# ryogrid/anime-illust-image-searcher

Measured on AMD Instinct MI355X. Metric: images/sec tagged (ViT fwd), higher is better.
Workload: dtype f16; 1 GPU; wd-tagger ViT-B/16 448px 16-bit-operand forward + sigmoid + MCut tag selection, batch 64 per GPU, u8 NHWC images resident in HBM (BASELINE.json configs[1]); batch_per_gpu=64, image=448x448x3 u8, classes=10861, parallelism=single GPU

## Files before the change

anime-illust-image-searcher_amd/csrc/vit.hip:

```cpp
#include <algorithm>
#include "../../include/hip_tagsearch_debug.h"
#include <cmath>
#include <cstdlib>
#include <cstdio>
#include <cstring>
#include <string>
#include <vector>

#include "vit_internal.h"
#include "model_host.h"

using namespace hipts;

namespace {

struct Layer {
    DevBuf ln1_g, ln1_b, ln2_g, ln2_b;
    DevBuf qkv_w, qkv_b, proj_w, proj_b, fc1_w, fc1_b, fc2_w, fc2_b;
    DevBuf qkv_u, qkv_c, fc1_u, fc1_c;
};


}

enum ProfCat { PC_PATCHIFY = 0, PC_GEMM_PATCH, PC_LAYERNORM, PC_GEMM_QK, PC_GEMM_VT, PC_ATTENTION, PC_GEMM_RESID,
               PC_GEMM_GELU, PC_POOL, PC_GEMM_HEAD, PC_OTHER, PC_COUNT };
static_assert(PC_COUNT == HIPTS_VIT_PROF_CATEGORIES, "category count");
static const char* const kProfNames[PC_COUNT] = {
    "patchify_kernel", "gemm_kernel<EPI_PATCH>", "layernorm_kernel", "gemm_kernel<EPI_QKV>", "gemm_kernel<EPI_VT>",
    "attn2_kernel", "gemm_kernel<EPI_RESID>", "gemm_kernel<EPI_GELU>", "pool_kernels", "gemm_kernel<EPI_HEAD>", "other"};

struct ProfRec {
    int cat;
    hipEvent_t a, b;
    double flops, bytes;
};

struct hipts_vit {
    bool prof = false;
    int prof_every = 0;
    uint32_t prof_mask = 0xffffffffu;
    long prof_calls = 0;
    std::vector<ProfRec> recs;
    std::vector<hipEvent_t> pool;
    double acc_ms[PC_COUNT] = {0}, acc_flops[PC_COUNT] = {0}, acc_bytes[PC_COUNT] = {0};
    int64_t acc_n[PC_COUNT] = {0};
    int device = 0;
    hipts_vit_config_t cfg{};
    int grid = 0, tokens = 0, tokens_pad = 0, patch_k = 0;
    std::vector<Layer> layers;
    DevBuf patch_w, patch_w2, patch_b, patch_b_u8, pos, norm_g, norm_b, head_w, head_b;
    std::vector<float> h_patch_bias, h_patch_rowsum;
    TensorLedger ledger;
    DevBuf img_in, a0, x, xn, q, k, v, att, hmid, pool_part, pooled2, logits, probs, stat_part;
    DevBuf x_rm;
    DevBuf sk_ws;
    bool fold_ln = false;
    bool fold_dirty = true;
    bool split_att = false;
    int pool_splits = 1;
    static constexpr int kMaxSub = 4;
    int want_sub = 0;
    bool deferred_join = false;
    int last_ns = 0;
    int pend_ns = 0, pend_batch = 0;
    SubStreams<kMaxSub> streams;
    hipEvent_t ev_stagger = nullptr;
};

namespace {

template <bool F16>
__global__ __launch_bounds__(256) void patchify_u8_kernel(const uint8_t* __restrict__ img, bf16_t* __restrict__ a0, int batch,
                                                          int size, int P, int grid) {
    const int64_t idx = (int64_t)blockIdx.x * 256 + threadIdx.x;
    const int64_t total = (int64_t)batch * grid * grid * P;
    if (idx >= total) return;
    const int ky = (int)(idx % P);
    const int64_t tok = idx / P;
    const int px = (int)(tok % grid), py = (int)((tok / grid) % grid), b = (int)(tok / ((int64_t)grid * grid));
    const uint8_t* src = img + (((int64_t)b * size + (py * P + ky)) * size + px * P) * 3;
    bf16_t* dst = a0 + tok * (int64_t)(P * P * 3) + ky * P * 3;
    if (P == 16) {
        const uint4* s4 = reinterpret_cast<const uint4*>(src);
        uint4* d4 = reinterpret_cast<uint4*>(dst);
#pragma unroll
        for (int v = 0; v < 3; ++v) {
            const uint4 in = s4[v];
            const uint32_t w[4] = {in.x, in.y, in.z, in.w};
            bf16x8 lo, hi;
#pragma unroll
            for (int e = 0; e < 8; ++e) {
                lo[e] = to_op<F16>((float)((w[e >> 2] >> (8 * (e & 3))) & 0xffu));
                hi[e] = to_op<F16>((float)((w[2 + (e >> 2)] >> (8 * (e & 3))) & 0xffu));
            }
            d4[2 * v] = *reinterpret_cast<const uint4*>(&lo);
            d4[2 * v + 1] = *reinterpret_cast<const uint4*>(&hi);
        }
        return;
    }
    for (int i = 0; i < P * 3; ++i) dst[i] = to_op<F16>((float)src[i]);
}

template <bool F16>
__global__ __launch_bounds__(256) void patchify_u8_p16_kernel(const uint8_t* __restrict__ img, bf16_t* __restrict__ a0, int size, int grid,
                                                              int xgroups) {
    __shared__ __attribute__((aligned(16))) char image[16 * 1536];
    const int tid = threadIdx.x;
    const int xg = blockIdx.x % xgroups, py = (blockIdx.x / xgroups) % grid, b = blockIdx.x / (xgroups * grid);
    const int px0 = xg * 16, ntok = min(16, grid - px0);
    const int chunks_per_row = ntok * 3;
    const int total = 16 * chunks_per_row;
    const uint8_t* src0 = img + (((int64_t)b * size + (int64_t)py * 16) * size + px0 * 16) * 3;
#pragma unroll
    for (int j = 0; j < 3; ++j) {
        const int L = j * 256 + tid;
        if (L < total) {
            const int ky = L / chunks_per_row, c16 = L - ky * chunks_per_row;
            const uint4 in = *reinterpret_cast<const uint4*>(src0 + (int64_t)ky * size * 3 + c16 * 16);
            const uint32_t w[4] = {in.x, in.y, in.z, in.w};
            bf16x8 lo, hi;
#pragma unroll
            for (int e = 0; e < 8; ++e) {
                lo[e] = to_op<F16>((float)((w[e >> 2] >> (8 * (e & 3))) & 0xffu));
                hi[e] = to_op<F16>((float)((w[2 + (e >> 2)] >> (8 * (e & 3))) & 0xffu));
            }
            const int tok = c16 / 3, part = c16 - tok * 3;
            char* d = image + tok * 1536 + ky * 96 + part * 32;
            *reinterpret_cast<bf16x8*>(d) = lo;
            *reinterpret_cast<bf16x8*>(d + 16) = hi;
        }
    }
    __syncthreads();
    const int out_chunks = ntok * 96;
    uint4* dst = reinterpret_cast<uint4*>(a0 + (((int64_t)b * grid + py) * grid + px0) * 768);
    for (int L = tid; L < out_chunks; L += 256) dst[L] = *reinterpret_cast<const uint4*>(image + L * 16);
}

template <bool F16>
__global__ __launch_bounds__(256) void patchify_f32_kernel(const float* __restrict__ x, bf16_t* __restrict__ a0, int batch,
                                                           int size, int P, int grid) {
    const int64_t idx = (int64_t)blockIdx.x * 256 + threadIdx.x;
    const int64_t total = (int64_t)batch * grid * grid * P;
    if (idx >= total) return;
    const int ky = (int)(idx % P);
    const int64_t tok = idx / P;
    const int px = (int)(tok % grid), py = (int)((tok / grid) % grid), b = (int)(tok / ((int64_t)grid * grid));
    const int K = P * P * 3;
    bf16_t* dst = a0 + tok * (int64_t)(2 * K) + ky * P * 3;
    for (int c = 0; c < 3; ++c) {
        const float* src = x + (((int64_t)b * 3 + (2 - c)) * size + (py * P + ky)) * size + px * P;
        for (int kx = 0; kx < P; ++kx) {
            const float v = src[kx];
            const bf16_t hi = to_op<F16>(v);
            dst[kx * 3 + c] = hi;
            dst[K + kx * 3 + c] = to_op<F16>(v - from_op<F16>(hi));
        }
    }
}

__device__ __forceinline__ float wave_sum(float v) {
#pragma unroll
    for (int o = 32; o >= 1; o >>= 1) v += __shfl_xor(v, o);
    return v;
}

template <bool F16, bool OUT8 = false>
__global__ __launch_bounds__(256) void layernorm_kernel(const float* __restrict__ x, const float* __restrict__ g,
                                                        const float* __restrict__ bta, bf16_t* __restrict__ out, int64_t rows,
                                                        int D, float eps) {
    const int lane = threadIdx.x & 63;
    const int64_t row = (int64_t)blockIdx.x * 4 + (threadIdx.x >> 6);
    if (row >= rows) return;
    const int nvec = D >> 2;
    const float4* xr = reinterpret_cast<const float4*>(x + row * D);
    float4 v[4];
    float s = 0.f;
#pragma unroll
    for (int i = 0; i < 4; ++i) {
        const int c = lane + 64 * i;
        v[i] = c < nvec ? xr[c] : make_float4(0.f, 0.f, 0.f, 0.f);
        s += (v[i].x + v[i].y) + (v[i].z + v[i].w);
    }
    const float mean = wave_sum(s) / (float)D;
    float ss = 0.f;
#pragma unroll
    for (int i = 0; i < 4; ++i) {
        if (lane + 64 * i < nvec) {
            const float a = v[i].x - mean, b = v[i].y - mean, c = v[i].z - mean, d = v[i].w - mean;
            ss += (a * a + b * b) + (c * c + d * d);
        }
    }
    const float rstd = 1.0f / sqrtf(wave_sum(ss) / (float)D + eps);
    const float4* gr = reinterpret_cast<const float4*>(g);
    const float4* br = reinterpret_cast<const float4*>(bta);
#pragma unroll
    for (int i = 0; i < 4; ++i) {
        const int c = lane + 64 * i;
        if (c < nvec) {
            const float4 gg = gr[c], bb = bta ? br[c] : make_float4(0.f, 0.f, 0.f, 0.f);
            if constexpr (OUT8)
                reinterpret_cast<uint32_t*>(reinterpret_cast<uint8_t*>(out) + row * D)[c] =
                    pack4_e4m3((v[i].x - mean) * rstd * gg.x + bb.x, (v[i].y - mean) * rstd * gg.y + bb.y,
                               (v[i].z - mean) * rstd * gg.z + bb.z, (v[i].w - mean) * rstd * gg.w + bb.w);
            else
            *reinterpret_cast<bf16x4*>(out + row * D + 4 * c) =
                pack4<F16>((v[i].x - mean) * rstd * gg.x + bb.x, (v[i].y - mean) * rstd * gg.y + bb.y,
                           (v[i].z - mean) * rstd * gg.z + bb.z, (v[i].w - mean) * rstd * gg.w + bb.w);
        }
    }
}

__global__ __launch_bounds__(256) void pool_partial_kernel(const float* __restrict__ x, float* __restrict__ part, int tokens,
                                                           int D, float eps, int normalize, int splits) {
    __shared__ float red[4][1024];
    const int lane = threadIdx.x & 63, wave = threadIdx.x >> 6;
    const int split = blockIdx.x, b = blockIdx.y;
    const int per = (tokens + splits - 1) / splits;
    const int t0 = split * per, t1 = min(tokens, t0 + per);
    const int nvec = D >> 2;
    float4 acc[4];
#pragma unroll
    for (int i = 0; i < 4; ++i) acc[i] = make_float4(0.f, 0.f, 0.f, 0.f);
    auto load_row = [&](int t, float4 (&v)[4]) {
        const float4* xr = reinterpret_cast<const float4*>(x + ((int64_t)b * tokens + (t < t1 ? t : t1 - 1)) * D);
#pragma unroll
        for (int i = 0; i < 4; ++i) {
            const int c = lane + 64 * i;
            v[i] = c < nvec ? xr[c] : make_float4(0.f, 0.f, 0.f, 0.f);
        }
    };
    float4 vn[4];
    if (t0 + wave < t1) load_row(t0 + wave, vn);
    for (int t = t0 + wave; t < t1; t += 4) {
        float4 v[4];
        float s = 0.f;
#pragma unroll
        for (int i = 0; i < 4; ++i) {
            v[i] = vn[i];
            s += (v[i].x + v[i].y) + (v[i].z + v[i].w);
        }
        if (t + 4 < t1) load_row(t + 4, vn);
        float mean = 0.f, rstd = 1.f;
        if (normalize) {
            mean = wave_sum(s) / (float)D;
            float ss = 0.f;
#pragma unroll
            for (int i = 0; i < 4; ++i)
                if (lane + 64 * i < nvec) {
                    const float a = v[i].x - mean, bq = v[i].y - mean, c = v[i].z - mean, d = v[i].w - mean;
                    ss += (a * a + bq * bq) + (c * c + d * d);
                }
            rstd = 1.0f / sqrtf(wave_sum(ss) / (float)D + eps);
        }
#pragma unroll
        for (int i = 0; i < 4; ++i) {
            acc[i].x += (v[i].x - mean) * rstd;
            acc[i].y += (v[i].y - mean) * rstd;
            acc[i].z += (v[i].z - mean) * rstd;
            acc[i].w += (v[i].w - mean) * rstd;
        }
    }
#pragma unroll
    for (int i = 0; i < 4; ++i) {
        const int c = lane + 64 * i;
        if (c < nvec) {
            red[wave][4 * c + 0] = acc[i].x;
            red[wave][4 * c + 1] = acc[i].y;
            red[wave][4 * c + 2] = acc[i].z;
            red[wave][4 * c + 3] = acc[i].w;
        }
    }
    __syncthreads();
    for (int d = threadIdx.x; d < D; d += 256)
        part[((int64_t)b * splits + split) * D + d] = (red[0][d] + red[1][d]) + (red[2][d] + red[3][d]);
}

template <bool F16>
__global__ __launch_bounds__(256) void pool_finalize_kernel(const float* __restrict__ part, const float* __restrict__ g,
                                                            const float* __restrict__ bta, bf16_t* __restrict__ out, int tokens,
                                                            int D, float eps, int normalize_after, int splits) {
    __shared__ float feat[1024];
    __shared__ float red[8];
    const int b = blockIdx.x;
    float s = 0.f;
    for (int d = threadIdx.x; d < D; d += 256) {
        float a = 0.f;
        for (int sp = 0; sp < splits; ++sp) a += part[((int64_t)b * splits + sp) * D + d];
        a = a / (float)tokens;
        feat[d] = a;
        s += a;
    }
    float mean = 0.f, rstd = 1.f;
    if (normalize_after) {
        s = wave_sum(s);
        if ((threadIdx.x & 63) == 0) red[threadIdx.x >> 6] = s;
        __syncthreads();
        mean = ((red[0] + red[1]) + (red[2] + red[3])) / (float)D;
        float ss = 0.f;
        for (int d = threadIdx.x; d < D; d += 256) {
            const float c = feat[d] - mean;
            ss += c * c;
        }
        ss = wave_sum(ss);
        if ((threadIdx.x & 63) == 0) red[4 + (threadIdx.x >> 6)] = ss;
        __syncthreads();
        rstd = 1.0f / sqrtf(((red[4] + red[5]) + (red[6] + red[7])) / (float)D + eps);
    }
    for (int d = threadIdx.x; d < D; d += 256) {
        const float f = (feat[d] - mean) * rstd * g[d] + bta[d];
        const bf16_t hi = to_op<F16>(f);
        const bf16_t lo = to_op<F16>(f - from_op<F16>(hi));
        out[(int64_t)b * 2 * D + d] = hi;
        out[(int64_t)b * 2 * D + D + d] = lo;
    }
}

}

extern "C" {

int hipts_vit_create(const hipts_vit_config_t* cfg, int device, hipts_vit_t** out) {
    HIPTS_REQUIRE(cfg && out, "hipts_vit_create: null argument");
    HIPTS_REQUIRE(cfg->patch >= 4 && cfg->image_size % cfg->patch == 0, "image_size must be a multiple of patch");
    HIPTS_REQUIRE(cfg->heads >= 1 && cfg->dim == cfg->heads * 64, "head dim must be 64 (dim = heads * 64)");
    HIPTS_REQUIRE(cfg->dim % 64 == 0 && cfg->dim <= 1024, "dim must be a multiple of 64, <= 1024");
    HIPTS_REQUIRE(cfg->mlp_dim % 64 == 0, "mlp_dim must be a multiple of 64");
    HIPTS_REQUIRE((cfg->patch * cfg->patch * 3) % 64 == 0, "patch*patch*3 must be a multiple of 64");
    HIPTS_REQUIRE(cfg->depth >= 1 && cfg->num_classes >= 1 && cfg->max_batch >= 1, "bad depth / classes / max_batch");
    const int grid = cfg->image_size / cfg->patch;
    HIPTS_REQUIRE((grid * grid) % 4 == 0, "token count must be a multiple of 4");
    HIPTS_TRY(use_device(device));
    auto* h = new hipts_vit();
    h->device = device;
    h->cfg = *cfg;
    h->grid = grid;
    h->tokens = grid * grid;
    h->tokens_pad = round_up(h->tokens, 64);
    h->patch_k = cfg->patch * cfg->patch * 3;
    h->split_att = (cfg->operand_f16 & HIPTS_OPERAND_SPLIT_ATT) != 0;
    h->layers.resize(cfg->depth);
    for (const char* s : {"patch_embed.proj.weight", "patch_embed.proj.bias", "pos_embed", "norm.weight", "norm.bias", "head.weight", "head.bias"})
        h->ledger.need(s);
    for (int i = 0; i < cfg->depth; ++i) {
        const std::string p = "blocks." + std::to_string(i) + ".";
        for (const char* s : {"norm1.weight", "norm1.bias", "attn.qkv.weight", "attn.qkv.bias", "attn.proj.weight",
                              "attn.proj.bias", "norm2.weight", "norm2.bias", "mlp.fc1.weight", "mlp.fc1.bias",
                              "mlp.fc2.weight", "mlp.fc2.bias"})
            h->ledger.need(p + s);
    }
    const size_t B = cfg->max_batch, M = B * h->tokens, D = cfg->dim;
    const size_t qkv_elems = B * cfg->heads * (size_t)h->tokens_pad * 64;
    h->pool_splits = h->tokens >= 64 ? std::min(32, std::max(8, h->tokens / 28)) : 1;
    if (getenv("HIPTS_POOL_SPLITS") && h->tokens >= 64) h->pool_splits = std::max(1, std::min(32, atoi(getenv("HIPTS_POOL_SPLITS"))));
    int st = HIPTS_OK;
    if ((st = h->a0.alloc(M * h->patch_k * 2 * 2)) || (st = h->x.alloc(M * D * 4)) || (st = h->x_rm.alloc(M * D * 4)) || (st = h->xn.alloc(M * D * 2)) ||
        (st = h->q.alloc(qkv_elems * 2)) || (st = h->k.alloc(qkv_elems * 2)) || (st = h->v.alloc(qkv_elems * 2)) ||
        (st = h->att.alloc(M * D * 2 * (h->split_att ? 2 : 1))) || (st = h->hmid.alloc(M * (size_t)cfg->mlp_dim * 2)) ||
        (st = h->pool_part.alloc(B * h->pool_splits * D * 4)) || (st = h->pooled2.alloc(B * 2 * D * 2)) ||
        (st = h->logits.alloc(B * (size_t)cfg->num_classes * 4)) || (st = h->probs.alloc(B * (size_t)cfg->num_classes * 4))) {
        delete h;
        return st;
    }
    h->fold_ln = D % 64 == 0 && h->tokens % 8 == 0 && cfg->mlp_dim % 8 == 0 && !getenv("HIPTS_GEMM") &&
                 !(getenv("HIPTS_LN_FOLD") && atoi(getenv("HIPTS_LN_FOLD")) == 0);
    if (h->fold_ln) {
        if ((st = h->stat_part.alloc(((D + 255) / 256) * M * 8))) {
            delete h;
            return st;
        }
        for (auto& L : h->layers)
            if ((st = L.qkv_u.alloc(3 * D * 4)) || (st = L.qkv_c.alloc(3 * D * 4)) || (st = L.fc1_u.alloc((size_t)cfg->mlp_dim * 4)) ||
                (st = L.fc1_c.alloc((size_t)cfg->mlp_dim * 4))) {
                delete h;
                return st;
            }
    }
    {
        hipError_t e2;
        if ((st = h->sk_ws.alloc(hipts_vit::kMaxSub * GEMM_SK_WS_BYTES)) || (e2 = hipMemset(h->sk_ws.p, 0, h->sk_ws.bytes)) != hipSuccess) {
            delete h;
            return st ? st : set_error(HIPTS_ERR_HIP, "hipMemset failed");
        }
    }
    hipError_t e;
    if ((e = hipMemset(h->q.p, 0, h->q.bytes)) != hipSuccess || (e = hipMemset(h->k.p, 0, h->k.bytes)) != hipSuccess ||
        (e = hipMemset(h->v.p, 0, h->v.bytes)) != hipSuccess) {
        delete h;
        return set_error(HIPTS_ERR_HIP, "hipMemset failed: %s", hipGetErrorString(e));
    }
    *out = h;
    return HIPTS_OK;
}

int hipts_vit_destroy(hipts_vit_t* h) {
    if (h) {
        (void)hipSetDevice(h->device);
        (void)hipDeviceSynchronize();
        if (h->ev_stagger) (void)hipEventDestroy(h->ev_stagger);
        delete h;
    }
    return HIPTS_OK;
}

int hipts_vit_set_tensor(hipts_vit_t* h, const char* key_c, const float* data, int64_t numel) {
    HIPTS_REQUIRE(h && key_c && data, "hipts_vit_set_tensor: null argument");
    HIPTS_TRY(use_device(h->device));
    const bool f16 = (h->cfg.operand_f16 & 1) != 0;
    const std::string key(key_c);
    const auto& c = h->cfg;
    const int D = c.dim, P = c.patch, Mlp = c.mlp_dim, C = c.num_classes;
#define EXPECT(n)                                                                                                      \
    HIPTS_REQUIRE(numel == (int64_t)(n), "tensor %s: expected %lld elements, got %lld", key_c, (long long)(n),         \
                  (long long)numel)
    int st = HIPTS_ERR_INVALID, li = 0;
    std::string sub;
    if (key == "patch_embed.proj.weight") {
        EXPECT((int64_t)D * 3 * P * P);
        std::vector<float> perm((size_t)D * h->patch_k);
        for (int n = 0; n < D; ++n)
            for (int ky = 0; ky < P; ++ky)
                for (int kx = 0; kx < P; ++kx)
                    for (int cr = 0; cr < 3; ++cr)
                        perm[(size_t)n * h->patch_k + (ky * P + kx) * 3 + cr] = data[(((size_t)n * 3 + (2 - cr)) * P + ky) * P + kx];
        st = upload_matrix16(h->patch_w, perm.data(), D, h->patch_k, round_up(D, 256), f16);
        if (st == HIPTS_OK) {
            h->h_patch_rowsum.assign(D, 0.f);
            for (int n = 0; n < D; ++n) {
                double rs = 0.0;
                for (int kk = 0; kk < h->patch_k; ++kk) {
                    float wv;
                    if (f16) {
                        wv = f16_bits_to_f32(f32_to_f16_rne(perm[(size_t)n * h->patch_k + kk]));
                    } else {
                        const uint32_t bits = (uint32_t)f32_to_bf16_rne(perm[(size_t)n * h->patch_k + kk]) << 16;
                        memcpy(&wv, &bits, 4);
                    }
                    rs += (double)wv;
                }
                h->h_patch_rowsum[n] = (float)rs;
            }
            st = upload_matrix16_dup(h->patch_w2, perm.data(), D, h->patch_k, round_up(D, 256), f16);
        }
    } else if (key == "patch_embed.proj.bias") {
        EXPECT(D);
        h->h_patch_bias.assign(data, data + D);
        st = upload_f32(h->patch_b, data, D);
    } else if (key == "pos_embed") {
        EXPECT((int64_t)h->tokens * D);
        st = upload_f32(h->pos, data, (size_t)h->tokens * D);
    } else if (key == "norm.weight") {
        EXPECT(D);
        st = upload_f32(h->norm_g, data, D);
    } else if (key == "norm.bias") {
        EXPECT(D);
        st = upload_f32(h->norm_b, data, D);
    } else if (key == "head.weight") {
        EXPECT((int64_t)C * D);
        st = upload_matrix16_dup(h->head_w, data, C, D, round_up(C, 256), f16);
    } else if (key == "head.bias") {
        EXPECT(C);
        st = upload_f32(h->head_b, data, C);
    } else if (parse_indexed(key, "blocks.", &li, &sub)) {
        HIPTS_REQUIRE(li >= 0 && li < c.depth, "tensor %s: block index out of range", key_c);
        Layer& L = h->layers[li];
        if (sub == "norm1.weight") { EXPECT(D); st = upload_f32(L.ln1_g, data, D); }
        else if (sub == "norm1.bias") { EXPECT(D); st = upload_f32(L.ln1_b, data, D); }
        else if (sub == "norm2.weight") { EXPECT(D); st = upload_f32(L.ln2_g, data, D); }
        else if (sub == "norm2.bias") { EXPECT(D); st = upload_f32(L.ln2_b, data, D); }
        else if (sub == "attn.qkv.weight") { EXPECT((int64_t)3 * D * D); st = upload_matrix16(L.qkv_w, data, 3 * D, D, round_up(2 * D, 256) + round_up(D, 256) + 256, f16); }
        else if (sub == "attn.qkv.bias") { EXPECT(3 * D); st = upload_f32(L.qkv_b, data, 3 * D); }
        else if (sub == "attn.proj.weight") {
            EXPECT((int64_t)D * D);
            if (h->split_att) {
                st = upload_matrix16_dup(L.proj_w, data, D, D, round_up(D, 256), f16, split_lo_scale(f16));
            } else {
                st = upload_matrix16(L.proj_w, data, D, D, round_up(D, 256), f16);
            }
        }
        else if (sub == "attn.proj.bias") { EXPECT(D); st = upload_f32(L.proj_b, data, D); }
        else if (sub == "mlp.fc1.weight") { EXPECT((int64_t)Mlp * D); st = upload_matrix16(L.fc1_w, data, Mlp, D, round_up(Mlp, 256), f16); }
        else if (sub == "mlp.fc1.bias") { EXPECT(Mlp); st = upload_f32(L.fc1_b, data, Mlp); }
        else if (sub == "mlp.fc2.weight") { EXPECT((int64_t)D * Mlp); st = upload_matrix16(L.fc2_w, data, D, Mlp, round_up(D, 256), f16); }
        else if (sub == "mlp.fc2.bias") { EXPECT(D); st = upload_f32(L.fc2_b, data, D); }
        else return set_error(HIPTS_ERR_INVALID, "unknown tensor key %s", key_c);
    } else {
        return set_error(HIPTS_ERR_INVALID, "unknown tensor key %s", key_c);
    }
#undef EXPECT
    if (st == HIPTS_OK) h->ledger.mark_set(key);
    if (st == HIPTS_OK) h->fold_dirty = true;
    if (st == HIPTS_OK && (key == "patch_embed.proj.weight" || key == "patch_embed.proj.bias") &&
        !h->h_patch_bias.empty() && !h->h_patch_rowsum.empty()) {
        std::vector<float> eff(D);
        for (int n = 0; n < D; ++n) eff[n] = (float)((double)h->h_patch_bias[n] - (double)h->h_patch_rowsum[n]);
        st = upload_f32(h->patch_b_u8, eff.data(), D);
    }
    return st;
}

int hipts_vit_profile_name(int category, char* buf, size_t n) {
    HIPTS_REQUIRE(buf && n > 0 && category >= 0 && category < PC_COUNT, "bad category");
    snprintf(buf, n, "%s", kProfNames[category]);
    return HIPTS_OK;
}

int hipts_vit_flops_per_image(const hipts_vit_t* h, double* flops) {
    HIPTS_REQUIRE(h && flops, "null argument");
    const double N = h->tokens, D = h->cfg.dim, Ml = h->cfg.mlp_dim, C = h->cfg.num_classes, Kp = h->patch_k;
    const double per_layer = 2 * N * D * 3 * D + 2 * 2 * N * N * D + 2 * N * D * D + 2 * 2 * N * D * Ml;
    *flops = 2 * N * Kp * D + h->cfg.depth * per_layer + 2 * D * C;
    return HIPTS_OK;
}

}

namespace {

struct ProfScope {
    hipts_vit* h;
    hipStream_t s;
    ProfRec r{};
    bool on;
    ProfScope(hipts_vit* h_, hipStream_t s_, int cat, double flops, double bytes) : h(h_), s(s_), on(h_->prof && ((h_->prof_mask >> cat) & 1u)) {
        if (!on) return;
        auto get = [&]() {
            hipEvent_t e;
            if (!h->pool.empty()) {
                e = h->pool.back();
                h->pool.pop_back();
            } else if (hipEventCreate(&e) != hipSuccess) {
                e = nullptr;
            }
            return e;
        };
        r.cat = cat;
        r.flops = flops;
        r.bytes = bytes;
        r.a = get();
        r.b = get();
        if (r.a) (void)hipEventRecord(r.a, s);
    }
    ~ProfScope() {
        if (!on) return;
        if (r.b) (void)hipEventRecord(r.b, s);
        h->recs.push_back(r);
    }
};

int prof_resolve(hipts_vit* h) {
    for (auto& r : h->recs) {
        if (r.a && r.b) {
            HIPTS_HIP(hipEventSynchronize(r.b));
            float ms = 0.f;
            HIPTS_HIP(hipEventElapsedTime(&ms, r.a, r.b));
            h->acc_ms[r.cat] += ms;
            h->acc_n[r.cat] += 1;
            h->acc_flops[r.cat] += r.flops;
            h->acc_bytes[r.cat] += r.bytes;
        }
        if (r.a) h->pool.push_back(r.a);
        if (r.b) h->pool.push_back(r.b);
    }
    h->recs.clear();
    return HIPTS_OK;
}

int vit_run_images(hipts_vit* h, const void* in_dev, bool is_u8, int i0, int nb, float* lg, float* pr, hipStream_t s, bool shared_chip,
                   int stagger_at = 0, int sub = 0) {
    const auto& c = h->cfg;
    const int D = c.dim, P = c.patch, S = c.image_size, T = h->tokens, Tp = h->tokens_pad, H = c.heads;
    const int M = nb * T;
    const bool f16 = (c.operand_f16 & 1) != 0;
    const size_t r0 = (size_t)i0 * T;
    const int a0_ld = is_u8 ? h->patch_k : 2 * h->patch_k;
    bf16_t* a0 = h->a0.as<bf16_t>() + r0 * a0_ld;
    float* x = h->x.as<float>() + r0 * D;
    float* x_rm = h->x_rm.as<float>() + r0 * D;
    bf16_t* xn = h->xn.as<bf16_t>() + r0 * D;
    const int att_k = h->split_att ? 2 * D : D;
    bf16_t* att = h->att.as<bf16_t>() + r0 * att_k;
    bf16_t* hmid = h->hmid.as<bf16_t>() + r0 * c.mlp_dim;
    const size_t qoff = (size_t)i0 * H * Tp * 64;
    bf16_t* q = h->q.as<bf16_t>() + qoff;
    bf16_t* k = h->k.as<bf16_t>() + qoff;
    bf16_t* v = h->v.as<bf16_t>() + qoff;
    float* pool_part = h->pool_part.as<float>() + (size_t)i0 * h->pool_splits * D;
    bf16_t* pooled2 = h->pooled2.as<bf16_t>() + (size_t)i0 * 2 * D;
    const size_t img_bytes = (size_t)S * S * 3 * (is_u8 ? 1 : 4);
    const char* in_p = (const char*)in_dev + (size_t)i0 * img_bytes;

    const double dM = (double)M, dD = (double)D, dMlp = (double)c.mlp_dim, dT = (double)T;
    {
        ProfScope ps(h, s, PC_PATCHIFY, 0.0, dM * h->patch_k * (is_u8 ? 3.0 : 6.0));
        const int64_t total = (int64_t)M * P;
        const int blocks = ceil_div(total, 256);
        if (is_u8 && P == 16 && (S * 3) % 16 == 0) {
            const int xgroups = (h->grid + 15) / 16;
            const int pblocks = nb * h->grid * xgroups;
            if (f16) patchify_u8_p16_kernel<true><<<pblocks, 256, 0, s>>>((const uint8_t*)in_p, a0, S, h->grid, xgroups);
            else patchify_u8_p16_kernel<false><<<pblocks, 256, 0, s>>>((const uint8_t*)in_p, a0, S, h->grid, xgroups);
        } else if (is_u8) {
            if (f16) patchify_u8_kernel<true><<<blocks, 256, 0, s>>>((const uint8_t*)in_p, a0, nb, S, P, h->grid);
            else patchify_u8_kernel<false><<<blocks, 256, 0, s>>>((const uint8_t*)in_p, a0, nb, S, P, h->grid);
        } else {
            if (f16) patchify_f32_kernel<true><<<blocks, 256, 0, s>>>((const float*)in_p, a0, nb, S, P, h->grid);
            else patchify_f32_kernel<false><<<blocks, 256, 0, s>>>((const float*)in_p, a0, nb, S, P, h->grid);
        }
        HIPTS_LAUNCH_CHECK();
    }
    GemmArgs g;
    g = GemmArgs{};
    g.f16 = f16;
    g.shared_chip = shared_chip;
    g.A = a0; g.M = M; g.N = D; g.out_f32 = x; g.pos = h->pos.as<float>(); g.tokens = T;
    if (is_u8) {
        g.W = h->patch_w.as<bf16_t>(); g.K = h->patch_k; g.bias = h->patch_b_u8.as<float>(); g.qscale = 2.0f / 255.0f;
    } else {
        g.W = h->patch_w2.as<bf16_t>(); g.K = 2 * h->patch_k; g.bias = h->patch_b.as<float>(); g.qscale = 1.0f;
    }
    const bool fold = h->fold_ln;
    static const bool xb_env = !(getenv("HIPTS_X_BLOCKED") && atoi(getenv("HIPTS_X_BLOCKED")) == 0);
    const bool xb = xb_env && fold && D % 16 == 0 && T % 16 == 0 && c.depth >= 1;
    const int sblocks = (D + 255) / 256;
    float* stat_p = fold ? h->stat_part.as<float>() + 2 * (size_t)sblocks * r0 : nullptr;
    {
        ProfScope ps(h, s, PC_GEMM_PATCH, 2.0 * dM * dD * h->patch_k, dM * h->patch_k * 2 + dM * dD * 4 + (fold ? dM * dD * 2 : 0.0));
        if (fold) {
            g.out_bf16 = xn; g.ln_gamma = h->layers[0].ln1_g.as<float>(); g.stat_part = stat_p; g.stat_stride = M;
            g.x_blocked = xb ? 1 : 0;
            HIPTS_TRY(launch_gemm(EPI_RESID_XG, g, s));
        } else {
            HIPTS_TRY(launch_gemm(EPI_PATCH, g, s));
        }
    }

    const int ln_blocks = ceil_div(M, 4);
    auto folded = [&](GemmArgs& ga, const float* u, const float* cvec) {
        ga.stat_in = stat_p; ga.stat_in_blocks = sblocks; ga.stat_in_stride = M; ga.ln_dim = D; ga.ln_eps = c.ln_eps;
        ga.col_u = u; ga.bias = cvec;
    };
    auto layernorm = [&](const float* gamma, const float* beta) -> int {
        ProfScope ps(h, s, PC_LAYERNORM, 0.0, dM * dD * 6);
        HIPTS_LAUNCH_F16(f16, layernorm_kernel, ln_blocks, 256, 0, s, x, gamma, beta, xn, M, D, c.ln_eps);
        return HIPTS_OK;
    };
    auto residual = [&](const bf16_t* A, const bf16_t* W, const float* bias, int K, const float* next_gamma, double flops, double bytes) -> int {
        GemmArgs r{};
        r.f16 = f16;
        r.shared_chip = shared_chip;
        r.A = A; r.W = W; r.M = M; r.N = D; r.K = K; r.bias = bias; r.out_f32 = x;
        r.sk_ws = h->sk_ws.as<char>() + (size_t)sub * GEMM_SK_WS_BYTES; r.sk_ws_bytes = GEMM_SK_WS_BYTES;
        r.x_blocked = xb ? 1 : 0;
        if (next_gamma) {
            r.out_bf16 = xn; r.ln_gamma = next_gamma; r.stat_part = stat_p; r.stat_stride = M;
        } else if (xb) {
            r.resid_rowmajor_out = x_rm;
        }
        {
            ProfScope ps(h, s, PC_GEMM_RESID, flops, bytes + (next_gamma ? dM * dD * 2 : 0.0));
            HIPTS_TRY(launch_gemm(next_gamma ? EPI_RESID_XG : EPI_RESID, r, s));
        }
        return HIPTS_OK;
    };
    for (int li = 0; li < c.depth; ++li) {
        Layer& L = h->layers[li];
        const bool ln1_folded = fold;
        if (!ln1_folded) HIPTS_TRY(layernorm(L.ln1_g.as<float>(), L.ln1_b.as<float>()));
        g = GemmArgs{};
        g.f16 = f16;
        g.shared_chip = shared_chip;
        g.A = xn; g.W = L.qkv_w.as<bf16_t>(); g.M = M; g.N = 3 * D; g.K = D;
        g.bias = L.qkv_b.as<float>(); g.out_bf16 = q; g.out2_bf16 = k; g.out3_bf16 = v;
        if (ln1_folded) folded(g, L.qkv_u.as<float>(), L.qkv_c.as<float>());
        g.tokens = T; g.tokens_pad = Tp; g.heads = H; g.dim = D;
        g.qscale = 0.125f * 1.4426950408889634f;
        {
            ProfScope ps(h, s, PC_GEMM_QK, 2.0 * dM * 3 * dD * dD, dM * dD * 2 + dM * 3 * dD * 2);
            HIPTS_TRY(launch_gemm(EPI_QK, g, s));
        }
        auto stagger = [&](int pos) {
            if (li == 0 && stagger_at == pos && h->ev_stagger) (void)hipEventRecord(h->ev_stagger, s);
        };
        stagger(1);
        {
            ProfScope ps(h, s, PC_ATTENTION, 4.0 * nb * H * dT * dT * 64, dM * dD * 2 * 4);
            HIPTS_TRY(launch_attention2(q, k, v, att, nb, H, T, Tp, f16, s, 0, 0, h->split_att ? 1 : 0, split_lo_scale(f16)));
        }
        stagger(2);
        HIPTS_TRY(residual(att, L.proj_w.as<bf16_t>(), L.proj_b.as<float>(), att_k, fold ? L.ln2_g.as<float>() : nullptr, 2.0 * dM * dD * att_k,
                           dM * att_k * 2 + dM * dD * 8));
        stagger(3);
        if (!fold) HIPTS_TRY(layernorm(L.ln2_g.as<float>(), L.ln2_b.as<float>()));
        g = GemmArgs{};
        g.f16 = f16;
        g.shared_chip = shared_chip;
        g.A = xn; g.W = L.fc1_w.as<bf16_t>(); g.M = M; g.N = c.mlp_dim; g.K = D;
        g.bias = L.fc1_b.as<float>(); g.out_bf16 = hmid; g.gelu_tanh = c.gelu_tanh;
        if (fold) folded(g, L.fc1_u.as<float>(), L.fc1_c.as<float>());
        {
            ProfScope ps(h, s, PC_GEMM_GELU, 2.0 * dM * dD * dMlp, dM * dD * 2 + dM * dMlp * 2);
            HIPTS_TRY(launch_gemm(EPI_GELU, g, s));
        }
        stagger(4);
        HIPTS_TRY(residual(hmid, L.fc2_w.as<bf16_t>(), L.fc2_b.as<float>(), c.mlp_dim,
                           (fold && li + 1 < c.depth) ? h->layers[li + 1].ln1_g.as<float>() : nullptr, 2.0 * dM * dD * dMlp,
                           dM * dMlp * 2 + dM * dD * 8));
        stagger(5);
    }
    {
        ProfScope ps(h, s, PC_POOL, 0.0, dM * dD * 4);
        pool_partial_kernel<<<dim3(h->pool_splits, nb), 256, 0, s>>>(xb ? x_rm : x, pool_part, T, D, c.ln_eps, c.pool_then_norm ? 0 : 1, h->pool_splits);
        HIPTS_LAUNCH_CHECK();
        if (f16)
            pool_finalize_kernel<true><<<nb, 256, 0, s>>>(pool_part, h->norm_g.as<float>(), h->norm_b.as<float>(), pooled2, T, D, c.ln_eps,
                                                          c.pool_then_norm ? 1 : 0, h->pool_splits);
        else
            pool_finalize_kernel<false><<<nb, 256, 0, s>>>(pool_part, h->norm_g.as<float>(), h->norm_b.as<float>(), pooled2, T, D, c.ln_eps,
                                                           c.pool_then_norm ? 1 : 0, h->pool_splits);
        HIPTS_LAUNCH_CHECK();
    }
    g = GemmArgs{};
    g.f16 = f16;
    g.shared_chip = shared_chip;
    g.A = pooled2; g.W = h->head_w.as<bf16_t>(); g.M = nb; g.N = c.num_classes; g.K = 2 * D;
    g.sk_ws = h->sk_ws.as<char>() + (size_t)sub * GEMM_SK_WS_BYTES; g.sk_ws_bytes = GEMM_SK_WS_BYTES;
    g.bias = h->head_b.as<float>(); g.out_f32 = lg ? lg + (size_t)i0 * c.num_classes : nullptr;
    g.out2_f32 = pr ? pr + (size_t)i0 * c.num_classes : nullptr;
    {
        ProfScope ps(h, s, PC_GEMM_HEAD, 2.0 * nb * dD * c.num_classes, (double)c.num_classes * 2 * dD * 2);
        HIPTS_TRY(launch_gemm(EPI_HEAD, g, s));
    }
    return HIPTS_OK;
}

int vit_forward_impl(hipts_vit* h, const void* input, int in_memspace, bool is_u8, int batch, float* logits_out,
                     float* probs_out, int out_memspace, hipStream_t s) {
    HIPTS_REQUIRE(h && input && batch >= 1, "hipts_vit_forward: bad arguments");
    HIPTS_REQUIRE(batch <= h->cfg.max_batch, "batch %d exceeds max_batch %d", batch, h->cfg.max_batch);
    HIPTS_TRY(h->ledger.require_complete("hipts_vit_forward"));
    HIPTS_TRY(use_device(h->device));
    h->prof = h->prof_every > 0 && (h->prof_calls++ % h->prof_every) == 0;
    const auto& c = h->cfg;
    const int S = c.image_size;

    static const int want_streams = getenv("HIPTS_VIT_STREAMS") ? atoi(getenv("HIPTS_VIT_STREAMS")) : 2;
    const int ns = std::min({h->want_sub > 0 ? h->want_sub : want_streams, (int)hipts_vit::kMaxSub, batch / 8});
    if (h->pend_ns > 0 && (h->pend_ns != ns || h->pend_batch != batch || in_memspace != HIPTS_DEVICE))
        for (int i = 0; i < h->pend_ns; ++i) HIPTS_HIP(hipStreamWaitEvent(s, h->streams.ev_join[i], 0));
    h->pend_ns = 0;

    const void* in_dev = nullptr;
    HIPTS_TRY(stage_input(h->img_in, input, in_memspace, (size_t)batch * S * S * 3 * (is_u8 ? 1 : 4), s, &in_dev));
    const bool dev_out = out_memspace == HIPTS_DEVICE;
    float* lg = (dev_out && logits_out) ? logits_out : h->logits.as<float>();
    float* pr = (probs_out || !dev_out) ? ((dev_out && probs_out) ? probs_out : h->probs.as<float>()) : nullptr;
    if (h->fold_ln && h->fold_dirty) {
        const bool f16w = (c.operand_f16 & 1) != 0;
        for (auto& L : h->layers) {
            HIPTS_TRY(launch_fold_ln(L.qkv_w.as<bf16_t>(), f16w, L.ln1_g.as<float>(), L.ln1_b.as<float>(), L.qkv_b.as<float>(), L.qkv_u.as<float>(),
                                     L.qkv_c.as<float>(), 3 * c.dim, c.dim, s));
            HIPTS_TRY(launch_fold_ln(L.fc1_w.as<bf16_t>(), f16w, L.ln2_g.as<float>(), L.ln2_b.as<float>(), L.fc1_b.as<float>(), L.fc1_u.as<float>(),
                                     L.fc1_c.as<float>(), c.mlp_dim, c.dim, s));
        }
        h->fold_dirty = false;
    }

    if (ns >= 2) {
        if (!h->streams.ev_fork) HIPTS_HIP(hipEventCreateWithFlags(&h->streams.ev_fork, hipEventDisableTiming));
        for (int i = 0; i < ns; ++i)
            if (!h->streams.sub[i]) {
                HIPTS_HIP(hipStreamCreateWithFlags(&h->streams.sub[i], hipStreamNonBlocking));
                if (!h->streams.ev_join[i]) HIPTS_HIP(hipEventCreateWithFlags(&h->streams.ev_join[i], hipEventDisableTiming));
            }
        HIPTS_HIP(hipEventRecord(h->streams.ev_fork, s));
        static const int stagger_at = getenv("HIPTS_VIT_STAGGER") ? atoi(getenv("HIPTS_VIT_STAGGER")) : 0;
        if (stagger_at > 0 && !h->ev_stagger) HIPTS_HIP(hipEventCreateWithFlags(&h->ev_stagger, hipEventDisableTiming));
        for (int i = 0; i < ns; ++i) {
            const int i0 = (int)((int64_t)batch * i / ns), i1 = (int)((int64_t)batch * (i + 1) / ns);
            HIPTS_HIP(hipStreamWaitEvent(h->streams.sub[i], h->streams.ev_fork, 0));
            if (i > 0 && stagger_at > 0) HIPTS_HIP(hipStreamWaitEvent(h->streams.sub[i], h->ev_stagger, 0));
            HIPTS_TRY(vit_run_images(h, in_dev, is_u8, i0, i1 - i0, lg, pr, h->streams.sub[i], true, i == 0 ? stagger_at : 0, i));
            HIPTS_HIP(hipEventRecord(h->streams.ev_join[i], h->streams.sub[i]));
            if (!h->deferred_join || !dev_out) HIPTS_HIP(hipStreamWaitEvent(s, h->streams.ev_join[i], 0));
        }
        h->last_ns = (h->deferred_join && dev_out) ? ns : 0;
        h->pend_ns = h->last_ns;
        h->pend_batch = batch;
    } else {
        HIPTS_TRY(vit_run_images(h, in_dev, is_u8, 0, batch, lg, pr, s, false));
        h->last_ns = 0;
        if (h->deferred_join && dev_out) {
            if (!h->streams.ev_join[0]) HIPTS_HIP(hipEventCreateWithFlags(&h->streams.ev_join[0], hipEventDisableTiming));
            HIPTS_HIP(hipEventRecord(h->streams.ev_join[0], s));
            h->last_ns = 1;
        }
    }
    if (!dev_out) HIPTS_TRY(read_back(s, (size_t)batch * c.num_classes * 4, logits_out, lg, probs_out, pr));
    return HIPTS_OK;
}

}

namespace hipts {
namespace {
__global__ __launch_bounds__(256) void rowstat_kernel(const float2* __restrict__ part, float2* __restrict__ rowstat, int M, int stride, int blocks,
                                                      int D, float eps) {
    const int q = threadIdx.x >> 6;
    const int m = blockIdx.x * 64 + (threadIdx.x & 63);
    __shared__ float2 red[4][64];
    float s1 = 0.f, s2 = 0.f;
    if (m < M) {
#pragma unroll 4
        for (int b = q; b < blocks; b += 4) {
            const float2 v = part[(size_t)b * stride + m];
            s1 += v.x;
            s2 += v.y;
        }
    }
    red[q][threadIdx.x & 63] = make_float2(s1, s2);
    __syncthreads();
    if (q != 0 || m >= M) return;
    const float2 a = red[0][threadIdx.x], b2 = red[1][threadIdx.x], c = red[2][threadIdx.x], d = red[3][threadIdx.x];
    s1 = (a.x + b2.x) + (c.x + d.x);
    s2 = (a.y + b2.y) + (c.y + d.y);
    const float mean = s1 / (float)D;
    const float var = fmaxf(s2 / (float)D - mean * mean, 0.f);
    const float rstd = 1.0f / sqrtf(var + eps);
    rowstat[m] = make_float2(rstd, rstd * mean);
}

template <bool F16>
__global__ __launch_bounds__(256) void fold_ln_kernel(const bf16_t* __restrict__ W, const float* __restrict__ gamma, const float* __restrict__ beta,
                                                      const float* __restrict__ bias, float* __restrict__ u, float* __restrict__ c, int N, int K) {
    const int lane = threadIdx.x & 63;
    const int n = blockIdx.x * 4 + (threadIdx.x >> 6);
    if (n >= N) return;
    double su = 0.0, sc = 0.0;
    for (int k = lane; k < K; k += 64) {
        const double w = (double)from_op<F16>(W[(size_t)n * K + k]);
        su += w * (double)gamma[k];
        if (beta) sc += w * (double)beta[k];
    }
#pragma unroll
    for (int o = 32; o >= 1; o >>= 1) {
        su += __shfl_xor(su, o);
        sc += __shfl_xor(sc, o);
    }
    if (lane == 0) {
        u[n] = (float)su;
        c[n] = (float)(sc + (bias ? (double)bias[n] : 0.0));
    }
}
}

int launch_rowstat(const float* part, float* rowstat, int M, int stride, int blocks, int D, float eps, hipStream_t s) {
    rowstat_kernel<<<(M + 63) / 64, 256, 0, s>>>(reinterpret_cast<const float2*>(part), reinterpret_cast<float2*>(rowstat), M, stride, blocks, D, eps);
    HIPTS_LAUNCH_CHECK();
    return HIPTS_OK;
}

int launch_fold_ln(const bf16_t* W, bool f16, const float* gamma, const float* beta, const float* bias, float* u, float* c, int N, int K,
                   hipStream_t s) {
    HIPTS_LAUNCH_F16(f16, fold_ln_kernel, (N + 3) / 4, 256, 0, s, W, gamma, beta, bias, u, c, N, K);
    return HIPTS_OK;
}

int launch_layernorm(const float* x, const float* g, const float* b, bf16_t* out, int64_t rows, int D, float eps, bool f16,
                     hipStream_t s) {
    HIPTS_REQUIRE(D % 4 == 0 && D >= 4 && D <= 1024, "layernorm: D=%d must be a multiple of 4, at most 1024", D);
    const int blocks = (int)((rows + 3) / 4);
    HIPTS_LAUNCH_F16(f16, layernorm_kernel, blocks, 256, 0, s, x, g, b, out, rows, D, eps);
    return HIPTS_OK;
}

int launch_layernorm8(const float* x, const float* g, const float* b, uint8_t* out, int64_t rows, int D, float eps, hipStream_t s) {
    HIPTS_REQUIRE(D % 4 == 0 && D >= 4 && D <= 1024, "layernorm: D=%d must be a multiple of 4, at most 1024", D);
    const int blocks = (int)((rows + 3) / 4);
    layernorm_kernel<true, true><<<blocks, 256, 0, s>>>(x, g, b, reinterpret_cast<bf16_t*>(out), rows, D, eps);
    HIPTS_LAUNCH_CHECK();
    return HIPTS_OK;
}
}

// ... 452 lines not shown
```

Baseline: 5411 images/sec.

## Fuse pool finalize via ticket, read blocked residual directly, add optional streaming head kernel

The pooling partial kernel can now read the tile-blocked residual layout directly, so the last residual GEMM no longer writes a separate row-major copy of x. It also runs the finalize step in the last-arriving block, using an atomic ticket per image, which removes one kernel launch. A new MFMA streaming head GEMM kernel is added behind an environment flag that is off by default. The atomic/ticket scheme adds synchronisation complexity and a reset dependency between calls.

```diff
diff --git a/anime-illust-image-searcher_amd/csrc/vit.hip b/anime-illust-image-searcher_amd/csrc/vit.hip
--- a/anime-illust-image-searcher_amd/csrc/vit.hip
+++ b/anime-illust-image-searcher_amd/csrc/vit.hip
@@ -59,6 +59,10 @@
     bool fold_dirty = true;
     bool split_att = false;
     int pool_splits = 1;
+    DevBuf pool_ticket;
+    bool pool_blocked = true;
+    bool pool_fused = true;
+    bool head_stream = false;
     static constexpr int kMaxSub = 4;
     int want_sub = 0;
     bool deferred_join = false;
@@ -211,9 +215,14 @@
     }
 }
 
+template <bool XBLK, bool FIN, bool F16>
 __global__ __launch_bounds__(256) void pool_partial_kernel(const float* __restrict__ x, float* __restrict__ part, int tokens,
-                                                           int D, float eps, int normalize, int splits) {
+                                                           int D, float eps, int normalize, int splits, unsigned* __restrict__ ticket,
+                                                           const float* __restrict__ g, const float* __restrict__ bta,
+                                                           bf16_t* __restrict__ out, int normalize_after) {
     __shared__ float red[4][1024];
+    __shared__ float fred[8];
+    __shared__ unsigned drawn;
     const int lane = threadIdx.x & 63, wave = threadIdx.x >> 6;
     const int split = blockIdx.x, b = blockIdx.y;
     const int per = (tokens + splits - 1) / splits;
@@ -223,7 +232,17 @@
 #pragma unroll
     for (int i = 0; i < 4; ++i) acc[i] = make_float4(0.f, 0.f, 0.f, 0.f);
     auto load_row = [&](int t, float4 (&v)[4]) {
-        const float4* xr = reinterpret_cast<const float4*>(x + ((int64_t)b * tokens + (t < t1 ? t : t1 - 1)) * D);
+        const int64_t m = (int64_t)b * tokens + (t < t1 ? t : t1 - 1);
+        if constexpr (XBLK) {
+            const float* xb = x + (((m >> 4) * (int64_t)(D >> 4)) << 8) + (m & 15) * 16;
+#pragma unroll
+            for (int i = 0; i < 4; ++i) {
+                const int c = lane + 64 * i;
+                v[i] = c < nvec ? *reinterpret_cast<const float4*>(xb + ((c >> 2) << 8) + (c & 3) * 4) : make_float4(0.f, 0.f, 0.f, 0.f);
+            }
+            return;
+        }
+        const float4* xr = reinterpret_cast<const float4*>(x + m * D);
 #pragma unroll
         for (int i = 0; i < 4; ++i) {
             const int c = lane + 64 * i;
@@ -272,8 +291,71 @@
         }
     }
     __syncthreads();
-    for (int d = threadIdx.x; d < D; d += 256)
-        part[((int64_t)b * splits + split) * D + d] = (red[0][d] + red[1][d]) + (red[2][d] + red[3][d]);
+    for (int d = threadIdx.x; d < D; d += 256) {
+        const float p = (red[0][d] + red[1][d]) + (red[2][d] + red[3][d]);
+        if constexpr (FIN) __hip_atomic_store(part + ((int64_t)b * splits + split) * D + d, p, __ATOMIC_RELAXED, __HIP_MEMORY_SCOPE_AGENT);
+        else part[((int64_t)b * splits + split) * D + d] = p;
+    }
+    if constexpr (FIN) {
+        asm volatile("s_waitcnt vmcnt(0)" ::: "memory");
+        __syncthreads();
+        if (threadIdx.x == 0) drawn = __hip_atomic_fetch_add(ticket + b, 1u, __ATOMIC_RELAXED, __HIP_MEMORY_SCOPE_AGENT);
+        __syncthreads();
+        if (drawn != (unsigned)(splits - 1)) return;
+        if (threadIdx.x == 0) __hip_atomic_store(ticket + b, 0u, __ATOMIC_RELAXED, __HIP_MEMORY_SCOPE_AGENT);
+        float* feat = red[0];
+        float s = 0.f;
+        float a4[4] = {0.f, 0.f, 0.f, 0.f};
+        const float* pb = part + (int64_t)b * splits * D;
+        for (int sp0 = 0; sp0 < splits; sp0 += 8) {
+            float v[8][4];
+#pragma unroll
+            for (int u = 0; u < 8; ++u)
+#pragma unroll
+                for (int j = 0; j < 4; ++j) {
+                    const int d = threadIdx.x + 256 * j;
+                    v[u][j] = (sp0 + u < splits && d < D) ? __hip_atomic_load(pb + (int64_t)(sp0 + u) * D + d, __ATOMIC_RELAXED, __HIP_MEMORY_SCOPE_AGENT) : 0.f;
+                }
+#pragma unroll
+            for (int u = 0; u < 8; ++u)
+                if (sp0 + u < splits) {
+#pragma unroll
+                    for (int j = 0; j < 4; ++j) a4[j] += v[u][j];
+                }
+        }
+#pragma unroll
+        for (int j = 0; j < 4; ++j) {
+            const int d = threadIdx.x + 256 * j;
+            if (d < D) {
+                const float a = a4[j] / (float)tokens;
+                feat[d] = a;
+                s += a;
+            }
+        }
+        float mean = 0.f, rstd = 1.f;
+        if (normalize_after) {
+            s = wave_sum(s);
+            if ((threadIdx.x & 63) == 0) fred[threadIdx.x >> 6] = s;
+            __syncthreads();
+            mean = ((fred[0] + fred[1]) + (fred[2] + fred[3])) / (float)D;
+            float ss = 0.f;
+            for (int d = threadIdx.x; d < D; d += 256) {
+                const float c = feat[d] - mean;
+                ss += c * c;
+            }
+            ss = wave_sum(ss);
+            if ((threadIdx.x & 63) == 0) fred[4 + (threadIdx.x >> 6)] = ss;
+            __syncthreads();
+            rstd = 1.0f / sqrtf(((fred[4] + fred[5]) + (fred[6] + fred[7])) / (float)D + eps);
+        }
+        for (int d = threadIdx.x; d < D; d += 256) {
+            const float f = (feat[d] - mean) * rstd * g[d] + bta[d];
+            const bf16_t hi = to_op<F16>(f);
+            const bf16_t lo = to_op<F16>(f - from_op<F16>(hi));
+            out[(int64_t)b * 2 * D + d] = hi;
+            out[(int64_t)b * 2 * D + D + d] = lo;
+        }
+    }
 }
 
 template <bool F16>
@@ -314,6 +396,75 @@
         out[(int64_t)b * 2 * D + d] = hi;
         out[(int64_t)b * 2 * D + D + d] = lo;
     }
+}
+
+
+template <bool F16, int MB>
+__global__ __launch_bounds__(128) void head_stream_kernel(const bf16_t* __restrict__ A, const bf16_t* __restrict__ W, const float* __restrict__ bias,
+                                                          float* __restrict__ logits, float* __restrict__ probs, int M, int N, int K,
+                                                          int w_rows) {
+    constexpr int AHEAD = 8;
+    const int lane = threadIdx.x & 63, wave = threadIdx.x >> 6;
+    const int r = lane & 15, q = lane >> 4;
+    const int nb0 = (blockIdx.x * 2 + wave) * 16;
+    if (nb0 >= N) return;
+    const int wrow = min(nb0 + r, w_rows - 1);
+    const bf16x8* wp = reinterpret_cast<const bf16x8*>(W + (size_t)wrow * K) + q;
+    const bf16x8* ap[MB];
+#pragma unroll
+    for (int i = 0; i < MB; ++i) ap[i] = reinterpret_cast<const bf16x8*>(A + (size_t)min(i * 16 + r, M - 1) * K) + q;
+    f32x4 acc[MB];
+#pragma unroll
+    for (int i = 0; i < MB; ++i) acc[i] = f32x4{0.f, 0.f, 0.f, 0.f};
+    const int ns = K >> 5;
+    bf16x8 wf[AHEAD], af[AHEAD][MB];
+#pragma unroll
+    for (int u = 0; u < AHEAD; ++u) {
+        wf[u] = __builtin_nontemporal_load(wp + 4 * u);
+#pragma unroll
+        for (int i = 0; i < MB; ++i) af[u][i] = ap[i][4 * u];
+    }
+    for (int s0 = AHEAD; s0 < ns; s0 += AHEAD) {
+#pragma unroll
+        for (int u = 0; u < AHEAD; ++u) {
+#pragma unroll
+            for (int i = 0; i < MB; ++i) acc[i] = mfma_16x16x32<F16>(wf[u], af[u][i], acc[i]);
+            wf[u] = __builtin_nontemporal_load(wp + 4 * (s0 + u));
+#pragma unroll
+            for (int i = 0; i < MB; ++i) af[u][i] = ap[i][4 * (s0 + u)];
+        }
+    }
+#pragma unroll
+    for (int u = 0; u < AHEAD; ++u)
+#pragma unroll
+        for (int i = 0; i < MB; ++i) acc[i] = mfma_16x16x32<F16>(wf[u], af[u][i], acc[i]);
+#pragma unroll
+    for (int i = 0; i < MB; ++i) {
+        const int m = i * 16 + r;
+        if (m >= M) continue;
+#pragma unroll
+        for (int e = 0; e < 4; ++e) {
+            const int n = nb0 + 4 * q + e;
+            if (n < N) {
+                const float v = acc[i][e] + bias[n];
+                if (logits) logits[(size_t)m * N + n] = v;
+                if (probs) probs[(size_t)m * N + n] = 1.0f / (1.0f + expf(-v));
+            }
+        }
+    }
+}
+
+template <bool F16>
+int launch_head_stream(const bf16_t* A, const bf16_t* W, const float* bias, float* logits, float* probs, int M, int N, int K, int w_rows, hipStream_t s) {
+    const int mb = (M + 15) / 16, grid = (N + 31) / 32;
+    switch (mb) {
+        case 1: head_stream_kernel<F16, 1><<<grid, 128, 0, s>>>(A, W, bias, logits, probs, M, N, K, w_rows); break;
+        case 2: head_stream_kernel<F16, 2><<<grid, 128, 0, s>>>(A, W, bias, logits, probs, M, N, K, w_rows); break;
+        case 3: head_stream_kernel<F16, 3><<<grid, 128, 0, s>>>(A, W, bias, logits, probs, M, N, K, w_rows); break;
+        default: head_stream_kernel<F16, 4><<<grid, 128, 0, s>>>(A, W, bias, logits, probs, M, N, K, w_rows); break;
+    }
+    HIPTS_LAUNCH_CHECK();
+    return HIPTS_OK;
 }
 
 }
@@ -353,8 +504,12 @@
     const size_t qkv_elems = B * cfg->heads * (size_t)h->tokens_pad * 64;
     h->pool_splits = h->tokens >= 64 ? std::min(32, std::max(8, h->tokens / 28)) : 1;
     if (getenv("HIPTS_POOL_SPLITS") && h->tokens >= 64) h->pool_splits = std::max(1, std::min(32, atoi(getenv("HIPTS_POOL_SPLITS"))));
+    auto env_on = [](const char* name) { return !(getenv(name) && atoi(getenv(name)) == 0); };
+    h->pool_blocked = env_on("HIPTS_POOL_BLOCKED");
+    h->pool_fused = env_on("HIPTS_POOL_FUSED");
+    h->head_stream = getenv("HIPTS_HEAD_STREAM") && atoi(getenv("HIPTS_HEAD_STREAM")) != 0;
     int st = HIPTS_OK;
-    if ((st = h->a0.alloc(M * h->patch_k * 2 * 2)) || (st = h->x.alloc(M * D * 4)) || (st = h->x_rm.alloc(M * D * 4)) || (st = h->xn.alloc(M * D * 2)) ||
+    if ((st = h->a0.alloc(M * h->patch_k * 2 * 2)) || (st = h->x.alloc(M * D * 4)) || (!h->pool_blocked && (st = h->x_rm.alloc(M * D * 4))) || (st = h->xn.alloc(M * D * 2)) ||
         (st = h->q.alloc(qkv_elems * 2)) || (st = h->k.alloc(qkv_elems * 2)) || (st = h->v.alloc(qkv_elems * 2)) ||
         (st = h->att.alloc(M * D * 2 * (h->split_att ? 2 : 1))) || (st = h->hmid.alloc(M * (size_t)cfg->mlp_dim * 2)) ||
         (st = h->pool_part.alloc(B * h->pool_splits * D * 4)) || (st = h->pooled2.alloc(B * 2 * D * 2)) ||
@@ -375,6 +530,12 @@
                 delete h;
                 return st;
             }
+    }
+    {
+        if ((st = h->pool_ticket.alloc(B * 4)) || hipMemset(h->pool_ticket.p, 0, h->pool_ticket.bytes) != hipSuccess) {
+            delete h;
+            return st ? st : set_error(HIPTS_ERR_HIP, "hipMemset failed");
+        }
     }
     {
         hipError_t e2;
@@ -576,7 +737,7 @@
     const int a0_ld = is_u8 ? h->patch_k : 2 * h->patch_k;
     bf16_t* a0 = h->a0.as<bf16_t>() + r0 * a0_ld;
     float* x = h->x.as<float>() + r0 * D;
-    float* x_rm = h->x_rm.as<float>() + r0 * D;
+    float* x_rm = h->x_rm.p ? h->x_rm.as<float>() + r0 * D : nullptr;
     bf16_t* xn = h->xn.as<bf16_t>() + r0 * D;
     const int att_k = h->split_att ? 2 * D : D;
     bf16_t* att = h->att.as<bf16_t>() + r0 * att_k;
@@ -654,7 +815,7 @@
         r.x_blocked = xb ? 1 : 0;
         if (next_gamma) {
             r.out_bf16 = xn; r.ln_gamma = next_gamma; r.stat_part = stat_p; r.stat_stride = M;
-        } else if (xb) {
+        } else if (xb && !h->pool_blocked) {
             r.resid_rowmajor_out = x_rm;
         }
         {
@@ -710,9 +871,23 @@
     }
     {
         ProfScope ps(h, s, PC_POOL, 0.0, dM * dD * 4);
-        pool_partial_kernel<<<dim3(h->pool_splits, nb), 256, 0, s>>>(xb ? x_rm : x, pool_part, T, D, c.ln_eps, c.pool_then_norm ? 0 : 1, h->pool_splits);
+        const bool pblk = xb && h->pool_blocked, pfin = h->pool_fused;
+        const dim3 pgrid(h->pool_splits, nb);
+        unsigned* ticket = h->pool_ticket.as<unsigned>() + i0;
+#define HIPTS_POOL_LAUNCH(XB, FIN, F)                                                                                                   \
+        pool_partial_kernel<XB, FIN, F><<<pgrid, 256, 0, s>>>(pblk ? x : (xb ? x_rm : x), pool_part, T, D, c.ln_eps, c.pool_then_norm ? 0 : 1, \
+                                                              h->pool_splits, ticket, h->norm_g.as<float>(), h->norm_b.as<float>(), pooled2, \
+                                                              c.pool_then_norm ? 1 : 0)
+        if (pfin) {
+            if (pblk) { if (f16) HIPTS_POOL_LAUNCH(true, true, true); else HIPTS_POOL_LAUNCH(true, true, false); }
+            else { if (f16) HIPTS_POOL_LAUNCH(false, true, true); else HIPTS_POOL_LAUNCH(false, true, false); }
+        } else {
+            if (pblk) HIPTS_POOL_LAUNCH(true, false, false); else HIPTS_POOL_LAUNCH(false, false, false);
+        }
+#undef HIPTS_POOL_LAUNCH
         HIPTS_LAUNCH_CHECK();
-        if (f16)
+        if (pfin) {
+        } else if (f16)
             pool_finalize_kernel<true><<<nb, 256, 0, s>>>(pool_part, h->norm_g.as<float>(), h->norm_b.as<float>(), pooled2, T, D, c.ln_eps,
                                                           c.pool_then_norm ? 1 : 0, h->pool_splits);
         else
@@ -729,7 +904,12 @@
     g.out2_f32 = pr ? pr + (size_t)i0 * c.num_classes : nullptr;
     {
         ProfScope ps(h, s, PC_GEMM_HEAD, 2.0 * nb * dD * c.num_classes, (double)c.num_classes * 2 * dD * 2);
-        HIPTS_TRY(launch_gemm(EPI_HEAD, g, s));
+        if (h->head_stream && nb <= 64 && g.K % 256 == 0) {
+            if (f16) HIPTS_TRY(launch_head_stream<true>(g.A, g.W, g.bias, g.out_f32, g.out2_f32, g.M, g.N, g.K, g.N, s));
+            else HIPTS_TRY(launch_head_stream<false>(g.A, g.W, g.bias, g.out_f32, g.out2_f32, g.M, g.N, g.K, g.N, s));
+        } else {
+            HIPTS_TRY(launch_gemm(EPI_HEAD, g, s));
+        }
     }
     return HIPTS_OK;
 }
```

New measurement: 5415 images/sec (median of 2 runs). No clear change (+0.1%).
